# amoretti86/PSVO

Hardware: AMD Instinct MI355X
Metric: particle-steps/sec (higher is better)
Workload: dtype f32

## Files before the change

### psvo_amd/csrc/bsim_bwd2_impl.h

```cpp
#pragma once
#define PSVO_BSIM_BWD_V2_UNIT 1
#include "bsim_bwd_impl.h"

namespace psvo {
PSVO_TIMERS_DEFINE(bsim_bwd2)

__device__ __forceinline__ float ldf(const float* base, unsigned off) {
    return *reinterpret_cast<const float*>(reinterpret_cast<const char*>(base) + off);
}
__device__ __forceinline__ int ldi(const int32_t* base, unsigned off) {
    return *reinterpret_cast<const int32_t*>(reinterpret_cast<const char*>(base) + off);
}
__device__ __forceinline__ void stf(float* base, unsigned off, float v) {
    *reinterpret_cast<float*>(reinterpret_cast<char*>(base) + off) = v;
}

__device__ __forceinline__ float swap_add32(float lo, float hi) {
    asm volatile("s_nop 1\n\tv_permlane32_swap_b32 %0, %1" : "+v"(lo), "+v"(hi));
    return lo + hi;
}
__device__ __forceinline__ float swap_add16(float lo, float hi) {
    asm volatile("s_nop 1\n\tv_permlane16_swap_b32 %0, %1" : "+v"(lo), "+v"(hi));
    return lo + hi;
}
// ... 4 lines not shown
    v += dpp_mov<0x121, 0xF, 0xF, true>(v, v);
    return v;
}

__device__ __forceinline__ float rs_bit3(float lo, float hi) {
    float r;
    asm volatile("s_nop 1\n\t"
                 "v_add_f32_dpp %0, %1, %1 row_ror:8 row_mask:0xf bank_mask:0x3\n\t"
                 "v_add_f32_dpp %0, %2, %2 row_ror:8 row_mask:0xf bank_mask:0xc"
                 : "=&v"(r) : "v"(lo), "v"(hi));
    return r;
}
__device__ __forceinline__ float rs_bit2(float lo, float hi) {
    float r;
    asm volatile("s_nop 1\n\t"
                 "v_add_f32_dpp %0, %1, %1 row_shl:4 row_mask:0xf bank_mask:0x5\n\t"
                 "v_add_f32_dpp %0, %2, %2 row_shr:4 row_mask:0xf bank_mask:0xa"
                 : "=&v"(r) : "v"(lo), "v"(hi));
    return r;
}
template <int K>
__device__ __forceinline__ void row_reduce_scatter(const float (&v)[4 * K], float (&out)[K]) {
    float h[2 * K];
#pragma unroll
    for (int i = 0; i < 2 * K; ++i) h[i] = rs_bit3(v[i], v[2 * K + i]);
#pragma unroll
    for (int i = 0; i < K; ++i) out[i] = group_sum<4>(rs_bit2(h[i], h[K + i]));
}

typedef float f4v __attribute__((ext_vector_type(4)));
typedef __bf16 bf8v __attribute__((ext_vector_type(8)));

__device__ __forceinline__ void bf16_split3(float v, unsigned& h, unsigned& m, unsigned& l) {
    const unsigned hb = __float_as_uint(v) & 0xffff0000u;
    const float r = v - __uint_as_float(hb);
    const unsigned mb = __float_as_uint(r) & 0xffff0000u;
    const float r2 = r - __uint_as_float(mb);
    h = hb >> 16;
    m = mb >> 16;
    l = __float_as_uint(r2) >> 16;
}
__device__ __forceinline__ uint4 bf16x3_a(float v) {
    unsigned h, m, l;
    bf16_split3(v, h, m, l);
    return make_uint4(h | (h << 16), m | (h << 16), l | (m << 16), m | (l << 16));
}
__device__ __forceinline__ uint4 bf16x3_b(float v) {
    unsigned h, m, l;
    bf16_split3(v, h, m, l);
    return make_uint4(h | (m << 16), h | (l << 16), h | (m << 16), l | (m << 16));
}

template <int DX, int DY, int H, int M, int JM>
__global__ void __launch_bounds__(256, 2) bsim_bwd2_kernel(const BsimBwdArgs a) {
    using MQ = MlpLds<DX, H, DX, 1>;
    using MG = MlpLds<DX, H, DY, 1>;
    using AC = BAcc<DX, DY>;
    constexpr int PS = (JM == 3) ? 20 : (DX == 4 && JM == 0) ? 5 : BTileSlot<DX>::kFloats;
    constexpr int FO = (JM == 3) ? 16 : 0;
    constexpr int NA = DX + 1;
    constexpr int PART = 2;
    constexpr int G = M * PART;
    constexpr int CPW = 64 / G;
    constexpr int CM = CPW * M;
    constexpr int NF = DX + 2;
    constexpr int UVS = (2 * DX + 3) & ~3;
    constexpr int JC = (JM == 0 && DX == 4) ? 2 : (JM || DX >= 3) ? 4 : 8;
    constexpr bool RO = (DX == 4) && (JM == 0);
    constexpr bool kSplitTile = (DX == 4) && (JM == 0);
    static_assert(CM == 32 && (M % 4) == 0, "two lanes per (chain, m): M in {4, 8, 16, 32}");
    extern __shared__ __attribute__((aligned(16))) float smem[];

    const int tid = threadIdx.x, lane = tid & 63, wave = tid >> 6;
    constexpr int NTB = 256, nwv = 4;
    const int B = a.B, T = a.T, N = a.N;
    const int NP = ((N + 127) / 128) * 128;
    const int nch = NP / (16 * JC);
    const int b = blockIdx.y, blk = blockIdx.x, nblk = gridDim.x;
    constexpr int cpb = nwv * CPW;
    const int cl = lane / G, part = (lane / M) & 1, m = lane % M;
    const bool h0 = (part == 0);
    const int n_raw = blk * cpb + wave * CPW + cl;
    const bool valid = n_raw < N;
    const int n = valid ? n_raw : N - 1;
    const bool srow = valid && h0;
    const bool lead = srow && (m == 0);
    const int j16 = lane & 15, g = lane >> 4;

    float* wf = smem;
    float* wg = wf + MQ::kSize;
    float* wqi = wg + MG::kSize;
    float* tile = wqi + MQ::kSize;
    float* jacc = tile + 2 * NP * PS;
    float* xch = jacc + nwv * NA * NP;
    float* uvx = xch + nwv * NF * CM;
    float* red = uvx + nwv * CM * UVS;
    float* const xw = xch + wave * NF * CM;
    float* const uw = uvx + wave * CM * UVS;
    float* const ja = jacc + wave * NA * NP;

    MQ::load(wf, a.f, tid, NTB);
    MG::load(wg, a.g, tid, NTB);
    MQ::load(wqi, a.q1inv, tid, NTB);

    const float kappa = sqrtf(0.5f * kLog2e);
    float isf[DX], rp[DX], isfk[DX], isg[DY];
#pragma unroll
    for (int d = 0; d < DX; ++d) {
        isf[d] = 1.f / a.sig_f[d];
        rp[d] = isf[d] * kappa;
        isfk[d] = isf[d] / kappa;
    }
    float ikap2 = 1.f / (kappa * kappa);
#pragma unroll
    for (int e = 0; e < DY; ++e) isg[e] = 1.f / a.sig_g[e];
    float pc[DX], pic[DX], pi1[DX], pi2[DX];
#pragma unroll
    for (int d = 0; d < DX; ++d) {
        pi1[d] = 1.f / a.sig_q1inv[d];
        pi2[d] = 1.f / a.sig_bq2[d];
        pic[d] = pi1[d] + pi2[d];
        pc[d] = 1.f / pic[d];
    }
    float s_init[DX], is_init[DX], i_isig[DX], im[DX], mi[DX];
#pragma unroll
    for (int d = 0; d < DX; ++d) {
        s_init[d] = a.sig_init[d];
        is_init[d] = 1.f / s_init[d];
        i_isig[d] = 1.f / a.isig[d];
        im[d] = a.imean[b * DX + d];
        mi[d] = a.minit[b * DX + d];
    }
    if constexpr (DX <= 2) {
        keep_in_vgpr(isf); keep_in_vgpr(rp); keep_in_vgpr(isfk); keep_in_vgpr(isg); keep_in_vgpr(ikap2);
        keep_in_vgpr(pc); keep_in_vgpr(pic); keep_in_vgpr(pi1); keep_in_vgpr(pi2);
    }
    const float ninf = -__builtin_huge_valf();
    const float aw = valid ? a.dscore[(size_t)b * N + n] : 0.f;

    const unsigned NM = (unsigned)N * M;
    unsigned o_nm = 4u * ((unsigned)b * NM + n * M + m);
    unsigned o_dnm[DX], o_knm[DY], o_dn[DX];
#pragma unroll
    for (int d = 0; d < DX; ++d) {
        o_dnm[d] = 4u * (((unsigned)b * DX + d) * NM + n * M + m);
        o_dn[d] = 4u * (((unsigned)b * DX + d) * N + n);
    }
#pragma unroll
    for (int k = 0; k < DY; ++k) o_knm[k] = 4u * (((unsigned)b * DY + k) * NM + n * M + m);
    unsigned o_n = 4u * ((unsigned)b * N + n);
    unsigned o_d = 4u * ((unsigned)b * DX), o_k = 4u * ((unsigned)b * DY);
    const unsigned s_nm = 4u * B * NM, s_dnm = s_nm * DX, s_knm = s_nm * DY, s_dn = 4u * B * DX * N, s_n = 4u * B * N,
                   s_d = 4u * B * DX, s_k = 4u * B * DY;

    float st[DX + 1], st_l = 0.f;
    int st_t = 0;
    auto put_slot = [&](float* buf, int j, const float (&raw)[DX + 1], float l) {
        float F[DX];
#pragma unroll
        for (int d = 0; d < DX; ++d) F[d] = raw[d] * rp[d];
        const float W = j < N ? (raw[DX] - l) * kLog2e : ninf;
        if constexpr (JM == 3) {
            const float Wf = fmaxf(W, -1e30f);
            uint4* q = reinterpret_cast<uint4*>(buf + j * PS);
            q[0] = bf16x3_b(F[0]);
            q[1] = bf16x3_b(F[DX > 1 ? 1 : 0]);
            q[2] = bf16x3_b(Wf - (F[0] * F[0] + F[DX > 1 ? 1 : 0] * F[DX > 1 ? 1 : 0]));
            q[3] = bf16x3_b(1.f);
            *reinterpret_cast<float4*>(buf + j * PS + 16) = make_float4(F[0], F[DX > 1 ? 1 : 0], 0.f, 0.f);
        } else if constexpr (JM == 2) {
            *reinterpret_cast<float4*>(buf + j * PS) = make_float4(F[0], F[1], W - (F[0] * F[0] + F[DX > 1 ? 1 : 0] * F[DX > 1 ? 1 : 0]), 1.f);
        } else if constexpr (DX <= 3) {
            float4 v;
            v.x = F[0];
            v.y = DX > 1 ? F[DX > 1 ? 1 : 0] : 0.f;
            v.z = DX > 2 ? F[DX > 2 ? 2 : 0] : 0.f;
            v.w = W;
            *reinterpret_cast<float4*>(buf + j * PS) = v;
        } else if constexpr (kSplitTile) {
            *reinterpret_cast<float4*>(buf + 4 * j) = make_float4(F[0], F[1], F[2], F[3]);
            buf[4 * NP + j] = W;
        } else {
            *reinterpret_cast<float4*>(buf + j * PS) = make_float4(F[0], F[1], F[2], F[3]);
            *reinterpret_cast<float4*>(buf + j * PS + 4) = make_float4(W, 0.f, 0.f, 0.f);
        }
    };
    auto tile_entry = [&](const float* buf, int j, float (&F)[DX], float& W) {
        if constexpr (kSplitTile) {
            const float4 e = *reinterpret_cast<const float4*>(buf + 4 * j);
            F[0] = e.x; F[DX > 1 ? 1 : 0] = e.y; F[DX > 2 ? 2 : 0] = e.z; F[DX > 3 ? 3 : 0] = e.w;
            W = buf[4 * NP + j];
        } else {
            read_slot<DX>(buf + j * PS, F, W);
        }
    };
    static_assert(offsetof(BsimBwdArgs, logW) - offsetof(BsimBwdArgs, Fm) == 8 &&
                  offsetof(BsimBwdArgs, lse) - offsetof(BsimBwdArgs, Fm) == 16 && offsetof(BsimBwdArgs, Fm) % 32 == 0,
                  "BsimBwdArgs: forward-tile pointer block");
    auto get_slot = [&](int tt, int j, float (&raw)[DX + 1], const float* Fm, const float* logW) {
        const unsigned tb = (unsigned)tt * B + b;
        const unsigned jc = j < N ? j : N - 1;
#pragma unroll
        for (int d = 0; d < DX; ++d) raw[d] = ldf(Fm, 4u * ((tb * DX + d) * N + jc));
        raw[DX] = ldf(logW, 4u * (tb * N + jc));
    };
    float st2[DX + 1];
    const bool two_slots = (DX >= 3) && NP > NTB;
    auto stage_load = [&](int tt) {
        unsigned long long pt[4];
        arg_block<4>((unsigned)offsetof(BsimBwdArgs, Fm), pt);
        st_t = tt;
        st_l = ldf(reinterpret_cast<const float*>(pt[2]), 4u * ((unsigned)tt * B + b));
        if (tid < NP) get_slot(tt, tid, st, reinterpret_cast<const float*>(pt[0]), reinterpret_cast<const float*>(pt[1]));
        if (two_slots && tid + NTB < NP)
            get_slot(tt, tid + NTB, st2, reinterpret_cast<const float*>(pt[0]), reinterpret_cast<const float*>(pt[1]));
    };
    auto stage_store = [&](float* buf) {
        if (tid < NP) put_slot(buf, tid, st, st_l);
        if (two_slots && tid + NTB < NP) put_slot(buf, tid + NTB, st2, st_l);
        for (int j = tid + (two_slots ? 2 : 1) * NTB; j < NP; j += NTB) {
            float raw[DX + 1];
            get_slot(st_t, j, raw, PSVO_ARG(BsimBwdArgs, Fm), PSVO_ARG(BsimBwdArgs, logW));
            put_slot(buf, j, raw, st_l);
        }
    };
    if (T >= 2) {
        stage_load(0);
        stage_store(tile);
    }
    __syncthreads();

    constexpr bool kAccLds = (DX >= 3);
    constexpr int kRowsA = 2 * DX + DY, kRowsB = 5 * DX, kSlotsB = 8;
    float acc[kAccLds ? 1 : AC::kN];
    float* const accA = red + 16 + wave * (kRowsA * 32 + kRowsB * kSlotsB);
    float* const accB = accA + kRowsA * 32;
    auto acc_is_lead = [](int k) { return k < 4 * DX || (k >= 5 * DX && k < 6 * DX); };
    auto acc_row = [](int k) {
        return k < 4 * DX ? k : k < 5 * DX ? k - 4 * DX : k < 6 * DX ? 4 * DX + (k - 5 * DX)
               : k < 7 * DX ? DX + (k - 6 * DX) : 2 * DX + (k - 7 * DX);
    };
    const int s32 = cl * M + m;
    if constexpr (kAccLds) {
        for (int i = lane; i < kRowsA * 32 + kRowsB * kSlotsB; i += 64) accA[i] = 0.f;
    } else {
#pragma unroll
        for (int i = 0; i < AC::kN; ++i) acc[i] = 0.f;
    }
    auto acc_add = [&](int k, float v) {
        if constexpr (kAccLds) {
            if (acc_is_lead(k)) atomicAdd(&accB[acc_row(k) * kSlotsB + cl], v);
            else atomicAdd(&accA[acc_row(k) * 32 + s32], v);
        } else {
            acc[k] += v;
        }
    };
    float dX[DX];
#pragma unroll
    for (int d = 0; d < DX; ++d) dX[d] = 0.f;

    struct StepIn {
        float eps[DX], bm[DX], xp[DX], mu1[DX], y[DY], om, lam2;
        int sel;
    };
    static_assert(offsetof(BsimBwdArgs, dscore) - offsetof(BsimBwdArgs, obs) == 56 && offsetof(BsimBwdArgs, obs) % 64 == 0 &&
                  offsetof(BsimBwdArgs, eps_b) - offsetof(BsimBwdArgs, obs) == 8 &&
                  offsetof(BsimBwdArgs, bwX) - offsetof(BsimBwdArgs, obs) == 16 &&
                  offsetof(BsimBwdArgs, sel) - offsetof(BsimBwdArgs, obs) == 24 &&
                  offsetof(BsimBwdArgs, lam2_all) - offsetof(BsimBwdArgs, obs) == 32 &&
                  offsetof(BsimBwdArgs, om_all) - offsetof(BsimBwdArgs, obs) == 40 &&
                  offsetof(BsimBwdArgs, mu1_all) - offsetof(BsimBwdArgs, obs) == 48, "BsimBwdArgs: input pointer block");
    auto load_step = [&](bool lst, bool fst, StepIn& s) {
        unsigned long long pb[8];
        arg_block<8>((unsigned)offsetof(BsimBwdArgs, obs), pb);
        const float* const p_obs = reinterpret_cast<const float*>(pb[0]);
        const float* const p_eps = reinterpret_cast<const float*>(pb[1]);
        const float* const p_bwX = reinterpret_cast<const float*>(pb[2]);
        const int32_t* const p_sel = reinterpret_cast<const int32_t*>(pb[3]);
        const float* const p_lam2 = reinterpret_cast<const float*>(pb[4]);
        const float* const p_om = reinterpret_cast<const float*>(pb[5]);
        const float* const p_mu1 = reinterpret_cast<const float*>(pb[6]);
        const float* const p_bm = PSVO_ARG(BsimBwdArgs, bmu2);
        s.sel = ldi(p_sel, o_n);
#pragma unroll
        for (int d = 0; d < DX; ++d) {
            s.eps[d] = ldf(p_eps, o_dnm[d]);
            s.bm[d] = ldf(p_bm, o_d + 4u * d);
            s.xp[d] = lst ? 0.f : ldf(p_bwX, o_dn[d] + s_dn);
            s.mu1[d] = lst ? 0.f : ldf(p_mu1, o_dn[d]);
        }
#pragma unroll
        for (int k = 0; k < DY; ++k) s.y[k] = ldf(p_obs, o_k + 4u * k);
        s.om = ldf(p_om, o_nm);
        s.lam2 = fst ? 0.f : ldf(p_lam2, o_nm);
    };
    auto advance = [&]() {
        o_nm += s_nm; o_n += s_n; o_d += s_d; o_k += s_k;
#pragma unroll
        for (int d = 0; d < DX; ++d) { o_dnm[d] += s_dnm; o_dn[d] += s_dn; }
#pragma unroll
        for (int k = 0; k < DY; ++k) o_knm[k] += s_knm;
    };
    StepIn cur_in, nxt_in;
    load_step(T == 1, true, cur_in);

    phase_skew(a.skew);
    SEC_INIT(bsim_bwd2)
    for (int t = 0; t < T; ++t) {
        SEC(0);
        const bool first = (t == 0), last = (t == T - 1);
        const float* cur = tile + ((t + 1) & 1) * NP * PS;
        float* nxt = tile + (t & 1) * NP * PS;
        constexpr bool kLateTile = (DX == 4);
        if (!kLateTile && t + 1 < T && t >= 1) stage_load(t);
        advance();
        constexpr bool kLatePrefetch = (DX >= 3);
        if (!kLatePrefetch && t + 1 < T) load_step(t + 2 == T, false, nxt_in);
        SEC(1);

        float xp[DX], eps[DX], bm[DX], mu1[DX], mu[DX], x[DX], y[DY];
        const int sel = cur_in.sel;
#pragma unroll
        for (int d = 0; d < DX; ++d) {
            eps[d] = cur_in.eps[d];
            bm[d] = cur_in.bm[d];
            xp[d] = cur_in.xp[d];
            mu1[d] = cur_in.mu1[d];
            if (!last) {
                mu[d] = pc[d] * fmaf(pi1[d], mu1[d], pi2[d] * bm[d]);
                x[d] = fmaf(pc[d], eps[d], mu[d]);
            } else {
                mu[d] = mi[d];
                x[d] = fmaf(s_init[d], eps[d], mu[d]);
            }
        }
#pragma unroll
        for (int k = 0; k < DY; ++k) y[k] = cur_in.y[k];
        const float pi_m = valid ? exp2_fast(cur_in.om * kLog2e) : 0.f;
        const float issel = (m == sel) ? 1.f : 0.f;
        const float dphi = aw * pi_m;
        const float dlam = -aw * (issel - pi_m);

        float dxt[DX];
#pragma unroll
        for (int d = 0; d < DX; ++d) dxt[d] = h0 ? issel * dX[d] : 0.f;

        SEC(2);
        if (!first) {
            if (h0) {
#pragma unroll
                for (int d = 0; d < DX; ++d) xw[d * CM + cl * M + m] = x[d] * rp[d];
                xw[DX * CM + cl * M + m] = cur_in.lam2;
                xw[(DX + 1) * CM + cl * M + m] = dlam;
            }
            __builtin_amdgcn_fence(__ATOMIC_RELEASE, "wavefront");
            __builtin_amdgcn_wave_barrier();
            __builtin_amdgcn_fence(__ATOMIC_ACQUIRE, "wavefront");

            if constexpr (RO) {
#pragma unroll 1
                for (int r = 0; r < 2; ++r) {
                    const int it4 = 4 * (4 * r + g);
                    f2 xa[DX], xb[DX], Ua[DX], Ub[DX], Va[DX], Vb[DX];
#pragma unroll
                    for (int d = 0; d < DX; ++d) {
                        const float4 v = *reinterpret_cast<const float4*>(xw + d * CM + it4);
                        xa[d] = f2{v.x, v.y};
                        xb[d] = f2{v.z, v.w};
                        Ua[d] = Ub[d] = Va[d] = Vb[d] = f2{0.f, 0.f};
                    }
                    const float4 lq = *reinterpret_cast<const float4*>(xw + DX * CM + it4);
                    const float4 dl = *reinterpret_cast<const float4*>(xw + (DX + 1) * CM + it4);
                    const f2 lqa = f2{lq.x, lq.y}, lqb = f2{lq.z, lq.w};
                    const f2 dla = f2{dl.x, dl.y}, dlb = f2{dl.z, dl.w};
#pragma unroll 1
                    for (int c = 0; c < nch; ++c) {
                        float A2[JC][NA];
#pragma unroll
                        for (int jt = 0; jt < JC; ++jt) {
                            float F[DX], W;
                            tile_entry(cur, (c * JC + jt) * 16 + j16, F, W);
                            f2 ua[DX], ub[DX], la = f2{W, W}, lb = la;
#pragma unroll
                            for (int d = 0; d < DX; ++d) {
                                const f2 Fd = f2{F[d], F[d]};
                                ua[d] = xa[d] - Fd;
                                ub[d] = xb[d] - Fd;
                                la = pk_fma(-ua[d], ua[d], la);
                                lb = pk_fma(-ub[d], ub[d], lb);
                            }
                            la -= lqa;
                            lb -= lqb;
                            const f2 pa = f2{exp2_fast(la.x), exp2_fast(la.y)}, pb = f2{exp2_fast(lb.x), exp2_fast(lb.y)};
                            const f2 ca = dla * pa, cb = dlb * pb;
#pragma unroll
                            for (int d = 0; d < DX; ++d) {
                                const f2 pua = pa * ua[d], pub = pb * ub[d];
                                Ua[d] += pua;
                                Ub[d] += pub;
                                Va[d] = pk_fma(pua, ua[d], Va[d]);
                                Vb[d] = pk_fma(pub, ub[d], Vb[d]);
                            }
                            const f2 cs = ca + cb;
                            A2[jt][DX] = cs.x + cs.y;
#pragma unroll
                            for (int d = 0; d < DX; ++d) {
                                const f2 ad = pk_fma(cb, ub[d], ca * ua[d]);
                                A2[jt][d] = ad.x + ad.y;
                            }
                        }
                        static_assert(JC == 2, "rounds-outer flush: two tiles per chunk");
#pragma unroll
                        for (int e = 0; e < NA; ++e) {
                            float v = swap_add32(A2[0][e], A2[1][e]);
                            v += xor_lane<16>(v);
                            if ((g & 1) == 0) {
                                float* dst = ja + e * NP + (c * JC + (g >> 1)) * 16 + j16;
                                *dst = (r == 0) ? v : *dst + v;
                            }
                        }
                    }
                    float vv[4 * 2 * DX], o[UVS];
#pragma unroll
                    for (int d = 0; d < DX; ++d) {
                        vv[0 * 2 * DX + d] = Ua[d].x; vv[1 * 2 * DX + d] = Ua[d].y;
                        vv[2 * 2 * DX + d] = Ub[d].x; vv[3 * 2 * DX + d] = Ub[d].y;
                        vv[0 * 2 * DX + DX + d] = Va[d].x; vv[1 * 2 * DX + DX + d] = Va[d].y;
                        vv[2 * 2 * DX + DX + d] = Vb[d].x; vv[3 * 2 * DX + DX + d] = Vb[d].y;
                    }
                    float red2[2 * DX];
                    row_reduce_scatter<2 * DX>(vv, red2);
#pragma unroll
                    for (int e = 0; e < UVS; ++e) o[e] = e < 2 * DX ? red2[e < 2 * DX ? e : 0] : 0.f;
                    if ((j16 & 3) == 0) {
                        float* dst = uw + (4 * (4 * r + g) + (j16 >> 2)) * UVS;
#pragma unroll
                        for (int e = 0; e < UVS; e += 4)
                            *reinterpret_cast<float4*>(dst + e) = make_float4(o[e], o[e + 1], o[e + 2], o[e + 3]);
                    }
                }
            } else {
            f2 Ua[2][DX], Ub[2][DX], Va[2][DX], Vb[2][DX];
#pragma unroll
            for (int r = 0; r < 2; ++r)
#pragma unroll
                for (int d = 0; d < DX; ++d) Ua[r][d] = Ub[r][d] = Va[r][d] = Vb[r][d] = f2{0.f, 0.f};

            for (int c = 0; c < nch; ++c) {
                float A2[JC][NA];
                f4v D4[JC];
#pragma unroll
                for (int jt = 0; jt < JC; ++jt) {
#pragma unroll
                    for (int e = 0; e < NA; ++e) A2[jt][e] = 0.f;
                    D4[jt] = f4v{0.f, 0.f, 0.f, 0.f};
                }
                const float* cbase = cur + (c * 16 * JC + j16) * PS;
#pragma unroll
                for (int r = 0; r < 2; ++r) {
                    const int it4 = 4 * (4 * r + g);
                    f2 xa[DX], xb[DX];
#pragma unroll
                    for (int d = 0; d < DX; ++d) {
                        const float4 v = *reinterpret_cast<const float4*>(xw + d * CM + it4);
                        xa[d] = f2{v.x, v.y};
                        xb[d] = f2{v.z, v.w};
                    }
                    const float4 lq = *reinterpret_cast<const float4*>(xw + DX * CM + it4);
                    const float4 dl = *reinterpret_cast<const float4*>(xw + (DX + 1) * CM + it4);
                    const f2 lqa = f2{lq.x, lq.y}, lqb = f2{lq.z, lq.w};
                    const f2 dla = f2{dl.x, dl.y}, dlb = f2{dl.z, dl.w};
// ... 57 lines not shown
                        }
                    } else
#pragma unroll
                    for (int jt = 0; jt < JC; ++jt) {
                        float F[DX], W;
                        if constexpr (kSplitTile) tile_entry(cur, (c * JC + jt) * 16 + j16, F, W);
                        else read_slot<DX>(cbase + jt * 16 * PS, F, W);
                        f2 ua[DX], ub[DX], la = f2{W, W}, lb = la;
#pragma unroll
                        for (int d = 0; d < DX; ++d) {
                            const f2 Fd = f2{F[d], F[d]};
                            ua[d] = xa[d] - Fd;
                            ub[d] = xb[d] - Fd;
                            la = pk_fma(-ua[d], ua[d], la);
                            lb = pk_fma(-ub[d], ub[d], lb);
                        }
                        la -= lqa;
                        lb -= lqb;
                        const f2 pa = f2{exp2_fast(la.x), exp2_fast(la.y)}, pb = f2{exp2_fast(lb.x), exp2_fast(lb.y)};
                        const f2 ca = dla * pa, cb = dlb * pb;
#pragma unroll
                        for (int d = 0; d < DX; ++d) {
                            const f2 pua = pa * ua[d], pub = pb * ub[d];
                            Ua[r][d] += pua;
                            Ub[r][d] += pub;
                            Va[r][d] = pk_fma(pua, ua[d], Va[r][d]);
                            Vb[r][d] = pk_fma(pub, ub[d], Vb[r][d]);
                        }
                        if constexpr (JM != 1) {
                            const f2 cs = ca + cb;
                            A2[jt][DX] += cs.x + cs.y;
#pragma unroll
                            for (int d = 0; d < DX; ++d) {
                                const f2 ad = pk_fma(cb, ub[d], ca * ua[d]);
                                A2[jt][d] += ad.x + ad.y;
                            }
                        } else {
                            D4[jt] = __builtin_amdgcn_mfma_f32_16x16x4f32(xop[0], ca.x, D4[jt], 0, 0, 0);
                            D4[jt] = __builtin_amdgcn_mfma_f32_16x16x4f32(xop[1], ca.y, D4[jt], 0, 0, 0);
                            D4[jt] = __builtin_amdgcn_mfma_f32_16x16x4f32(xop[2], cb.x, D4[jt], 0, 0, 0);
                            D4[jt] = __builtin_amdgcn_mfma_f32_16x16x4f32(xop[3], cb.y, D4[jt], 0, 0, 0);
                        }
                    }
                }
                if constexpr (JM != 1) {
                    float v[JC][NA];
#pragma unroll
                    for (int jt = 0; jt < JC; ++jt)
#pragma unroll
                        for (int e = 0; e < NA; ++e) v[jt][e] = A2[jt][e];
#pragma unroll
                    for (int jt = 0; jt < JC / 2; ++jt)
#pragma unroll
                        for (int e = 0; e < NA; ++e) v[jt][e] = swap_add32(v[jt][e], v[jt + JC / 2][e]);
#pragma unroll
                    for (int jt = 0; jt < JC / 4; ++jt)
#pragma unroll
                        for (int e = 0; e < NA; ++e) v[jt][e] = swap_add16(v[jt][e], v[jt + JC / 4][e]);
                    const int jt0 = (JC / 2) * (g >> 1) + (JC / 4) * (g & 1);
#pragma unroll
                    for (int jt = 0; jt < JC / 4; ++jt) {
                        if constexpr (JM >= 2) {
                            const float2 F2 = *reinterpret_cast<const float2*>(cbase + (jt0 + jt) * 16 * PS + FO);
                            v[jt][0] = fmaf(-F2.x, v[jt][DX], v[jt][0]);
                            v[jt][DX > 1 ? 1 : 0] = fmaf(-F2.y, v[jt][DX], v[jt][DX > 1 ? 1 : 0]);
                        }
#pragma unroll
                        for (int e = 0; e < NA; ++e) ja[e * NP + (c * JC + jt0 + jt) * 16 + j16] = v[jt][e];
                    }
                } else {
                    if (g == 0 || DX > 3) {
#pragma unroll
                        for (int jt = 0; jt < JC; ++jt) {
                            float F[DX], W;
                            read_slot<DX>(cbase + jt * 16 * PS, F, W);
                            (void)W;
                            const int j = (c * JC + jt) * 16 + j16;
                            if constexpr (DX <= 3) {
                                const float sc = D4[jt][DX];
#pragma unroll
                                for (int d = 0; d < DX; ++d) ja[d * NP + j] = D4[jt][d] - F[d] * sc;
                                ja[DX * NP + j] = sc;
                            } else {
                                const float sc = __shfl(D4[jt][0], 16 + j16);
                                if (g == 0) {
#pragma unroll
                                    for (int d = 0; d < DX; ++d) ja[d * NP + j] = D4[jt][d] - F[d] * sc;
                                    ja[DX * NP + j] = sc;
                                }
                            }
                        }
                    }
                }
            }
#pragma unroll
            for (int r = 0; r < 2; ++r) {
                float vv[4 * 2 * DX], o[UVS];
#pragma unroll
                for (int d = 0; d < DX; ++d) {
                    vv[0 * 2 * DX + d] = Ua[r][d].x; vv[1 * 2 * DX + d] = Ua[r][d].y;
                    vv[2 * 2 * DX + d] = Ub[r][d].x; vv[3 * 2 * DX + d] = Ub[r][d].y;
                    vv[0 * 2 * DX + DX + d] = Va[r][d].x; vv[1 * 2 * DX + DX + d] = Va[r][d].y;
                    vv[2 * 2 * DX + DX + d] = Vb[r][d].x; vv[3 * 2 * DX + DX + d] = Vb[r][d].y;
                }
                float red2[2 * DX];
                row_reduce_scatter<2 * DX>(vv, red2);
#pragma unroll
                for (int e = 0; e < UVS; ++e) o[e] = e < 2 * DX ? red2[e < 2 * DX ? e : 0] : 0.f;
                if ((j16 & 3) == 0) {
                    float* dst = uw + (4 * (4 * r + g) + (j16 >> 2)) * UVS;
#pragma unroll
                    for (int e = 0; e < UVS; e += 4)
                        *reinterpret_cast<float4*>(dst + e) = make_float4(o[e], o[e + 1], o[e + 2], o[e + 3]);
                }
            }
            }
            __builtin_amdgcn_fence(__ATOMIC_RELEASE, "wavefront");
            __builtin_amdgcn_wave_barrier();
            __builtin_amdgcn_fence(__ATOMIC_ACQUIRE, "wavefront");
            SEC(3);
            if (h0) {
                float uv[UVS];
#pragma unroll
                for (int e = 0; e < UVS; e += 4) {
                    const float4 q4 = *reinterpret_cast<const float4*>(uw + (cl * M + m) * UVS + e);
                    uv[e] = q4.x; uv[e + 1] = q4.y; uv[e + 2] = q4.z; uv[e + 3] = q4.w;
                }
                if constexpr (JM >= 2) {
#pragma unroll
                    for (int d = 0; d < DX; ++d) {
                        const float xs = x[d] * rp[d], r1 = uv[d], r2 = uv[DX + d];
                        uv[d] = xs - r1;
                        uv[DX + d] = fmaf(xs, xs - 2.f * r1, r2);
                    }
                }
#pragma unroll
                for (int d = 0; d < DX; ++d) {
                    dxt[d] -= dlam * uv[d] * isfk[d];
                    acc_add(AC::kSf + d, dlam * (uv[DX + d] * ikap2 - 1.f) * isf[d]);
                }
            }
        } else {
#pragma unroll
            for (int d = 0; d < DX; ++d) {
                const float z = (x[d] - im[d]) * i_isig[d];
                const float tz = dphi * z * i_isig[d];
                if (h0) {
                    dxt[d] -= tz;
                    acc_add(AC::kSiota + d, dphi * (z * z - 1.f) * i_isig[d]);
                }
            }
        }

        if (kLatePrefetch && t + 1 < T) load_step(t + 2 == T, false, nxt_in);
        if (kLateTile && t + 1 < T && t >= 1) stage_load(t);
        SEC(4);
        float dxp_part[DX];
#pragma unroll
        for (int d = 0; d < DX; ++d) dxp_part[d] = 0.f;
        {
            float dFo[DX];
#pragma unroll
            for (int d = 0; d < DX; ++d) dFo[d] = 0.f;
            if (!last) {
                float fmx[DX];
                MQ::template eval_part<PART>(wf, part, x, fmx);
#pragma unroll
                for (int d = 0; d < DX; ++d) fmx[d] += xor_lane<M>(fmx[d]);
#pragma unroll
                for (int d = 0; d < DX; ++d) {
                    const float z = (xp[d] - fmx[d]) * isf[d];
                    dFo[d] = dphi * z * isf[d];
                    if (h0) {
                        dxp_part[d] = -dFo[d];
                        acc_add(AC::kSf + d, dphi * (z * z - 1.f) * isf[d]);
                    }
                }
                MQ::template bwd_input_part<PART>(wf, part, x, dFo, dxt);
            }
            static_assert(offsetof(BsimBwdArgs, dFt) - offsetof(BsimBwdArgs, xt) == 8 &&
                          offsetof(BsimBwdArgs, dGt) - offsetof(BsimBwdArgs, xt) == 16 &&
                          offsetof(BsimBwdArgs, dmu1) - offsetof(BsimBwdArgs, xt) == 24 && offsetof(BsimBwdArgs, xt) % 32 == 0,
                          "BsimBwdArgs: row pointer block");
            unsigned long long pr[4];
            arg_block<4>((unsigned)offsetof(BsimBwdArgs, xt), pr);
            if (srow) {
#pragma unroll
                for (int d = 0; d < DX; ++d) {
                    stf(reinterpret_cast<float*>(pr[1]), o_dnm[d] - s_dnm, dFo[d]);
                    stf(reinterpret_cast<float*>(pr[0]), o_dnm[d] - s_dnm, x[d]);
                }
            }
            float gm[DY], dGo[DY];
            MG::template eval_part<PART>(wg, part, x, gm);
#pragma unroll
            for (int k = 0; k < DY; ++k) gm[k] += xor_lane<M>(gm[k]);
#pragma unroll
            for (int k = 0; k < DY; ++k) {
                float dmean = 1.f;
                if (a.emission) { dmean = emis_dmean(gm[k]); gm[k] = emis_mean(gm[k]); }
                const float z = (y[k] - gm[k]) * isg[k];
                dGo[k] = dphi * z * isg[k] * dmean;
                if (h0) acc_add(AC::kSg + k, dphi * (z * z - 1.f) * isg[k]);
                if (srow) stf(reinterpret_cast<float*>(pr[2]), o_knm[k] - s_knm, dGo[k]);
            }
            MG::template bwd_input_part<PART>(wg, part, x, dGo, dxt);
        }

        SEC(5);
        float dmu[DX], sce[DX], dxp[DX], dim[DX];
#pragma unroll
        for (int d = 0; d < DX; ++d) {
            const float v3 = (first && h0) ? dphi * (x[d] - im[d]) * i_isig[d] * i_isig[d] : 0.f;
            dmu[d] = group_sum<G>(dxt[d]);
            sce[d] = group_sum<G>(dxt[d] * eps[d]);
            dxp[d] = group_sum<G>(dxp_part[d]);
            dim[d] = first ? group_sum<G>(v3) : 0.f;
        }
        float outv[DX];
        if (!last) {
            float dmu1[DX];
#pragma unroll
            for (int d = 0; d < DX; ++d) {
                dmu1[d] = dmu[d] * pc[d] * pi1[d];
                outv[d] = dmu[d] * pc[d] * pi2[d];
                if (lead) {
                    stf(PSVO_ARG(BsimBwdArgs, dmu1), o_dn[d] - s_dn, dmu1[d]);
                    acc_add(AC::kSc + d, sce[d] + aw * pic[d]);
                    acc_add(AC::kSmm1 + d, dmu[d] * mu1[d]);
                    acc_add(AC::kSmb + d, dmu[d] * bm[d]);
                    acc_add(AC::kSmm + d, dmu[d] * mu[d]);
                }
            }
            {
                constexpr int kQS = (H / 4 < G) ? H / 4 : G;
                float dq[DX];
#pragma unroll
                for (int d = 0; d < DX; ++d) dq[d] = 0.f;
                MQ::template bwd_input_part<kQS>(wqi, (lane % G) & (kQS - 1), xp, dmu1, dq);
#pragma unroll
                for (int d = 0; d < DX; ++d) dxp[d] += group_sum<kQS>(dq[d]);
            }
        } else {
#pragma unroll
            for (int d = 0; d < DX; ++d) {
                outv[d] = dmu[d];
                if (lead) {
                    stf(PSVO_ARG(BsimBwdArgs, dmu1), o_dn[d] - s_dn, 0.f);
                    acc_add(AC::kSinit + d, sce[d] + aw * is_init[d]);
                }
            }
        }
#pragma unroll
        for (int d = 0; d < DX; ++d) dX[d] = dxp[d];
        if (lead) {
#pragma unroll
            for (int d = 0; d < DX; ++d) {
                stf(PSVO_ARG(BsimBwdArgs, dbmu2_rows), o_dn[d] - s_dn, last ? 0.f : outv[d]);
                if (last) PSVO_ARG(BsimBwdArgs, dminit_rows)[((size_t)b * DX + d) * N + n] = outv[d];
                if (first) PSVO_ARG(BsimBwdArgs, dimean_rows)[((size_t)b * DX + d) * N + n] = dim[d];
            }
        }
        SEC(6);
        __syncthreads();
        const size_t tb = (size_t)t * B + b;
        if (!first) {
            const size_t tbm = tb - B;
            float* const pF = PSVO_ARG(BsimBwdArgs, dFm_part) + (tbm * nblk + blk) * DX * N;
            float* const pW = PSVO_ARG(BsimBwdArgs, dlogW_part) + (tbm * nblk + blk) * N;
            for (int j = tid; j < N; j += NTB) {
#pragma unroll
                for (int d = 0; d < NA; ++d) {
                    const float* col = jacc + d * NP + j;
                    const float a0 = col[0], a1 = col[NA * NP], a2 = col[2 * NA * NP], a3 = col[3 * NA * NP];
                    const float s = (a0 + a1) + (a2 + a3);
                    if (d < DX) pF[d * N + j] = s * isfk[d < DX ? d : 0];
                    else pW[j] = s;
                }
            }
        }
        if (last) {
            float* const pF = PSVO_ARG(BsimBwdArgs, dFm_part) + (tb * nblk + blk) * DX * N;
            float* const pW = PSVO_ARG(BsimBwdArgs, dlogW_part) + (tb * nblk + blk) * N;
            for (int j = tid; j < N; j += NTB) {
#pragma unroll
                for (int d = 0; d < DX; ++d) pF[d * N + j] = 0.f;
                pW[j] = 0.f;
            }
        }
        SEC(7);
        if (t + 1 < T && t >= 1) stage_store(nxt);
        cur_in = nxt_in;
        __syncthreads();
        SEC(8);
    }

    for (int i = 0; i < AC::kN; ++i) {
        float v = 0.f;
        if constexpr (kAccLds) {
            if (acc_is_lead(i)) v = lane < kSlotsB ? accB[acc_row(i) * kSlotsB + lane] : 0.f;
            else v = lane < 32 ? accA[acc_row(i) * 32 + lane] : 0.f;
        } else {
#pragma unroll
            for (int k = 0; k < AC::kN; ++k) v = (k == i) ? acc[k] : v;
        }
        v = wave_sum(v);
        if (lane == 0) red[wave] = v;
        __syncthreads();
        if (tid == 0) {
            float s = 0.f;
            for (int w = 0; w < nwv; ++w) s += red[w];
            a.sacc_part[((size_t)b * nblk + blk) * AC::kN + i] = s;
        }
        __syncthreads();
    }
}

static inline void bsim2_geometry(int N, int M, int& cpb, int& nblk) {
    cpb = 4 * (64 / (2 * M));
    nblk = (N + cpb - 1) / cpb;
}

static inline bool bsim2_supported(int B, int T, int N, int M, int Dx, int Dy) {
    if (pick_m(M, [](auto) { return PSVO_OK; }) != PSVO_OK) return false;
    const long long big = (long long)T * B * (Dx > Dy ? Dx : Dy) * N * M * 4;
    return big < (1ll << 32);
}

template <int DX, int DY, int H, int M>
static int launch_bsim_bwd2(const BsimBwdArgs& a, const BsimBwdOut& o, int jm, hipStream_t stream) {
    using MQ = MlpLds<DX, H, DX, 1>;
    using MG = MlpLds<DX, H, DY, 1>;
    const int PS = (jm == 3 && DX == 2) ? 20 : (DX == 4) ? 5 : BTileSlot<DX>::kFloats;
    constexpr int UVS = (2 * DX + 3) & ~3;
    int cpb, nblk;
    bsim2_geometry(a.N, M, cpb, nblk);
    const int NP = ((a.N + 127) / 128) * 128;
    const size_t lds = sizeof(float) * (2 * MQ::kSize + MG::kSize + 2 * (size_t)NP * PS + 4 * (size_t)(DX + 1) * NP +
                                        4 * (DX + 2) * 32 + 4 * 32 * UVS + 16 +
                                        (DX >= 3 ? 4 * ((2 * DX + DY) * 32 + 5 * DX * 8) : 0));
    if (lds > 160 * 1024) return PSVO_ERR_UNSUPPORTED;
    BsimBwdArgs as = a;
    as.skew = (int)(2560.0 * NP / 128.0 * (3 * DX + 4) / 10.0 * g_tune_skew_pct / 100.0);
    clear_hip_error();
    if (jm == 3 && DX == 2) {
        if constexpr (DX == 2)
            hipLaunchKernelGGL((bsim_bwd2_kernel<DX, DY, H, M, 3>), dim3(nblk, a.B), dim3(256), lds, stream, as);
    } else if (jm == 2 && DX == 2) {
        if constexpr (DX == 2)
            hipLaunchKernelGGL((bsim_bwd2_kernel<DX, DY, H, M, 2>), dim3(nblk, a.B), dim3(256), lds, stream, as);
    } else if (jm == 1 && DX == 2) {
        if constexpr (DX == 2)
            hipLaunchKernelGGL((bsim_bwd2_kernel<DX, DY, H, M, 1>), dim3(nblk, a.B), dim3(256), lds, stream, as);
    } else {
        hipLaunchKernelGGL((bsim_bwd2_kernel<DX, DY, H, M, 0>), dim3(nblk, a.B), dim3(256), lds, stream, as);
    }
    (void)o;
    return launch_status();
}

template <int DX>
int bb2_dispatch_dy(const BsimBwdArgs& a, const BsimBwdOut& o, int Dy, int H, int M, int jm, hipStream_t s) {
    return dispatch_dy_h_m(Dy, H, M, [&](auto dy, auto h, auto m) __attribute__((visibility("hidden"))) {
        return launch_bsim_bwd2<DX, dy(), h(), m()>(a, o, jm, s); });
}

}
```

### psvo_amd/csrc/common.h

```cpp
#pragma once
#include <cstddef>
#include <type_traits>
#include <hip/hip_runtime.h>
#include <stdint.h>

#include "../../include/psvo_hip.h"

#ifndef PSVO_L
#define PSVO_L 1
#endif
#if PSVO_L == 1
#define PSVO_LNS l1
#define PSVO_ENTRY(name) extern "C" int name
#define PSVO_L2_DECL(name) extern "C" __attribute__((visibility("hidden"))) decltype(name) name##_l2;
#elif PSVO_L == 2
#define PSVO_LNS l2
#define PSVO_ENTRY(name) extern "C" __attribute__((visibility("hidden"))) int name##_l2
#define PSVO_L2_DECL(name)
#else
#error "PSVO_L must be 1 or 2"
#endif

namespace psvo {

constexpr float kLog2e = 1.4426950408889634f;
constexpr float kLn2 = 0.6931471805599453f;
constexpr float kHalfLog2Pi = 0.9189385332046727f;
constexpr int kWave = 64;

extern thread_local hipError_t g_last_hip_error;
inline void clear_hip_error() { (void)hipGetLastError(); }
inline int launch_status() {
    const hipError_t e = hipGetLastError();
    if (e != hipSuccess) g_last_hip_error = e;
    return e == hipSuccess ? PSVO_OK : PSVO_ERR_HIP;
}

inline bool desc_layers_ok(const psvo_desc* d) { return !d || (d->layers >= 0 && d->layers <= 2); }

extern int g_tune_l2_split;
extern int g_tune_filter_bwd_scan;

extern int g_tune_skew_pct;

__device__ __forceinline__ void phase_skew(int cycles) {
    unsigned hw;
    asm volatile("s_getreg_b32 %0, hwreg(HW_REG_HW_ID)" : "=s"(hw));
    if (cycles > 0 && ((hw >> 16) & 1u)) {
        for (int i = 0; i < cycles; i += 64 * 32) __builtin_amdgcn_s_sleep(32);
    }
}

inline bool mlp_layers_ok(const psvo_mlp* m) { return PSVO_L == 1 || !m || (m->Wh && m->bh); }

template <int V, int... Vs, class F>
static inline int pick(int v, F&& f) {
    if (v == V) return f(std::integral_constant<int, V>{});
    if constexpr (sizeof...(Vs) > 0) return pick<Vs...>(v, f);
    else return PSVO_ERR_UNSUPPORTED;
}
template <class F> static inline int pick_dx(int Dx, F&& f) { return pick<2, 3, 4>(Dx, f); }
template <class F> static inline int pick_dy(int Dy, F&& f) { return pick<1, 2>(Dy, f); }
template <class F> static inline int pick_m(int M, F&& f) { return pick<4, 8, 16, 32>(M, f); }
inline namespace PSVO_LNS {
template <class F> static inline int pick_h(int H, F&& f) {
#if PSVO_L == 1
    return pick<16, 32, 64>(H, f);
#else
    return pick<32, 64>(H, f);
#endif
}

template <class F> static inline int dispatch_dy_h(int Dy, int H, F&& f) {
    return pick_dy(Dy, [&](auto dy) { return pick_h(H, [&](auto h) { return f(dy, h); }); });
}
template <class F> static inline int dispatch_dy_h_m(int Dy, int H, int M, F&& f) {
    return dispatch_dy_h(Dy, H, [&](auto dy, auto h) { return pick_m(M, [&](auto m) { return f(dy, h, m); }); });
}
template <class F> static inline int dispatch_shape(int Dx, int Dy, int H, F&& f) {
    return pick_dx(Dx, [&](auto dx) { return dispatch_dy_h(Dy, H, [&](auto dy, auto h) { return f(dx, dy, h); }); });
}
template <class F> static inline int dispatch_shape_m(int Dx, int Dy, int H, int M, F&& f) {
    return pick_dx(Dx, [&](auto dx) { return dispatch_dy_h_m(Dy, H, M, [&](auto dy, auto h, auto m) { return f(dx, dy, h, m); }); });
}
}

static inline int wr_cluster(int B, int N, int M) {
    int K = 8;
    while (K > 1 && ((long long)B * K > 256 || N < 4 * K || (N + K - 1) / K * (K - 1) >= N)) K >>= 1;
    (void)M;
    return K;
}

#ifdef PSVO_SECTION_TIMERS
#define PSVO_TIMERS_DEFINE(name)                                                                        \
    __device__ unsigned long long g_sec_##name[32];                                                       \
    extern "C" int psvo_debug_timers_##name(unsigned long long* out, int reset) {                         \
        if (hipMemcpyFromSymbol(out, HIP_SYMBOL(g_sec_##name), 32 * sizeof(unsigned long long)) != hipSuccess) \
            return -1;                                                                                    \
        if (reset) {                                                                                      \
            unsigned long long z[32] = {0};                                                               \
            if (hipMemcpyToSymbol(HIP_SYMBOL(g_sec_##name), z, sizeof(z)) != hipSuccess) return -1;       \
        }                                                                                                 \
        return 0;                                                                                         \
    }
#define SEC_INIT(name)                                                                          \
    unsigned long long* const _sec = g_sec_##name;                                              \
    const bool _rec = (blockIdx.x == 0 && blockIdx.y == 0 && threadIdx.x == 0);                 \
    unsigned long long _tp = clock64();
#define SEC(i)                                   \
    do {                                         \
        const unsigned long long _tn = clock64(); \
        if (_rec) _sec[i] += _tn - _tp;          \
        _tp = _tn;                               \
    } while (0)
#else
#define PSVO_TIMERS_DEFINE(name)
#define SEC_INIT(name)
#define SEC(i)
#endif

__device__ __forceinline__ float exp2_fast(float x) { return __builtin_amdgcn_exp2f(x); }
__device__ __forceinline__ float log2_fast(float x) { return __builtin_amdgcn_logf(x); }

typedef float f2 __attribute__((ext_vector_type(2)));
__device__ __forceinline__ f2 pk_fma(f2 a, f2 b, f2 c) { return __builtin_elementwise_fma(a, b, c); }
__device__ __forceinline__ f2 pk_max(f2 a, f2 b) { return __builtin_elementwise_max(a, b); }
template <int HALF>
__device__ __forceinline__ f2 pk_fma_bcast(f2 a, f2 b, f2 c) {
    f2 d;
    if constexpr (HALF == 0)
        asm("v_pk_fma_f32 %0, %1, %2, %3 op_sel_hi:[0,1,1]" : "=v"(d) : "v"(a), "v"(b), "v"(c));
    else
        asm("v_pk_fma_f32 %0, %1, %2, %3 op_sel:[1,0,0] op_sel_hi:[1,1,1]" : "=v"(d) : "v"(a), "v"(b), "v"(c));
    return d;
}

__device__ __forceinline__ void keep_in_vgpr(float& x) { asm volatile("" : "+v"(x)); }
template <int K>
__device__ __forceinline__ void keep_in_vgpr(float (&x)[K]) {
#pragma unroll
    for (int i = 0; i < K; ++i) asm volatile("" : "+v"(x[i]));
}

template <class T>
__device__ __forceinline__ T* arg_ptr(unsigned byte_off) {
    asm volatile("" : "+s"(byte_off));
    typedef const char __attribute__((address_space(4))) * kptr;
    const kptr kp = (kptr)__builtin_amdgcn_kernarg_segment_ptr();
    typedef T* const __attribute__((address_space(4))) * pptr;
    return *(pptr)(kp + byte_off);
}
template <int NPTR>
__device__ __forceinline__ void arg_block(unsigned byte_off, unsigned long long (&out)[NPTR]) {
    static_assert(NPTR == 2 || NPTR == 4 || NPTR == 8, "pointer block of 2, 4 or 8");
    asm volatile("" : "+s"(byte_off));
    typedef const char __attribute__((address_space(4))) * kptr;
    const kptr kp = (kptr)__builtin_amdgcn_kernarg_segment_ptr();
    typedef unsigned long long vec_t __attribute__((ext_vector_type(NPTR)));
    typedef const vec_t __attribute__((address_space(4))) * vptr;
    const vec_t v = *(vptr)(kp + byte_off);
#pragma unroll
    for (int i = 0; i < NPTR; ++i) out[i] = v[i];
}
#define PSVO_ARG(args_type, field) \
    ::psvo::arg_ptr<std::remove_pointer_t<decltype(args_type::field)>>((unsigned)offsetof(args_type, field))

__device__ __forceinline__ float emis_mean(float r) { return (r > 20.f ? r : log1pf(expf(r))) + 1e-6f; }
__device__ __forceinline__ float emis_dmean(float r) { return 1.f / (1.f + expf(-r)); }

template <int DIN, int H, int DOUT, int L = 1>
struct MlpLds;

template <int DIN, int H, int DOUT>
struct MlpLds<DIN, H, DOUT, 1> {
    static constexpr int kW1 = 0;
    static constexpr int kB1 = DIN * H;
    static constexpr int kW2 = kB1 + H;
    static constexpr int kB2 = kW2 + DOUT * H;
    static constexpr int kSize = kB2 + ((DOUT + 3) & ~3);

    __device__ static void load(float* __restrict__ w, const psvo_mlp& p, int tid, int nthreads) {
        for (int i = tid; i < DIN * H; i += nthreads) w[kW1 + i] = p.W1[i];
        for (int i = tid; i < H; i += nthreads) w[kB1 + i] = p.b1[i];
        for (int i = tid; i < DOUT * H; i += nthreads) {
            const int o = i / H, k = i - o * H;
            w[kW2 + i] = p.W2[k * DOUT + o];
        }
        for (int i = tid; i < ((DOUT + 3) & ~3); i += nthreads) w[kB2 + i] = i < DOUT ? p.b2[i] : 0.f;
    }

    __device__ __forceinline__ static void group4(const float* __restrict__ w, int k, const float (&x)[DIN],
                                                  f2 (&acc)[DOUT]) {
        const float4 b = *reinterpret_cast<const float4*>(w + kB1 + k);
        f2 ha = f2{b.x, b.y}, hb = f2{b.z, b.w};
#pragma unroll
        for (int i = 0; i < DIN; ++i) {
            const float4 wi = *reinterpret_cast<const float4*>(w + kW1 + i * H + k);
            const f2 xi = f2{x[i], x[i]};
            ha = pk_fma(xi, f2{wi.x, wi.y}, ha);
            hb = pk_fma(xi, f2{wi.z, wi.w}, hb);
        }
        const f2 zero = f2{0.f, 0.f};
        ha = pk_max(ha, zero);
        hb = pk_max(hb, zero);
#pragma unroll
        for (int o = 0; o < DOUT; ++o) {
            const float4 wo = *reinterpret_cast<const float4*>(w + kW2 + o * H + k);
            acc[o] = pk_fma(ha, f2{wo.x, wo.y}, acc[o]);
            acc[o] = pk_fma(hb, f2{wo.z, wo.w}, acc[o]);
        }
    }

    template <bool ROLLED = false>
    __device__ __forceinline__ static void eval(const float* __restrict__ w, const float (&x)[DIN],
                                                float (&out)[DOUT]) {
        f2 acc[DOUT];
#pragma unroll
        for (int o = 0; o < DOUT; ++o) acc[o] = f2{w[kB2 + o], 0.f};
        if constexpr (ROLLED && (H % 8 == 0) && (H > 8)) {
#pragma unroll 1
            for (int k = 0; k < H; k += 8) {
                group4(w, k, x, acc);
                group4(w, k + 4, x, acc);
            }
        } else {
#pragma unroll
            for (int k = 0; k < H; k += 4) group4(w, k, x, acc);
        }
#pragma unroll
        for (int o = 0; o < DOUT; ++o) out[o] = acc[o].x + acc[o].y;
    }

    template <int S, int PB = 0>
    __device__ __forceinline__ static void eval_part(const float* __restrict__ w, int part, const float (&x)[DIN],
                                                     float (&out)[DOUT]) {
        constexpr int HP = H / S;
        static_assert(HP % 4 == 0, "hidden slice must be a multiple of 4");
        const float* wp = w + part * HP;
        f2 acc[DOUT];
#pragma unroll
        for (int o = 0; o < DOUT; ++o) acc[o] = f2{part == 0 ? w[kB2 + o] : 0.f, 0.f};
#pragma unroll
        for (int k = 0; k < HP; k += 4) group4(wp, k, x, acc);
#pragma unroll
        for (int o = 0; o < DOUT; ++o) out[o] = acc[o].x + acc[o].y;
    }

    __device__ __forceinline__ static void bwd_group4(const float* __restrict__ w, int k, const float (&x)[DIN],
                                                      const float (&dout)[DOUT], f2 (&dxa)[DIN]) {
        const float4 b = *reinterpret_cast<const float4*>(w + kB1 + k);
        f2 pa = f2{b.x, b.y}, pb = f2{b.z, b.w};
        f2 wa[DIN], wb[DIN];
#pragma unroll
        for (int i = 0; i < DIN; ++i) {
            const float4 wi = *reinterpret_cast<const float4*>(w + kW1 + i * H + k);
            wa[i] = f2{wi.x, wi.y};
            wb[i] = f2{wi.z, wi.w};
            const f2 xi = f2{x[i], x[i]};
            pa = pk_fma(xi, wa[i], pa);
            pb = pk_fma(xi, wb[i], pb);
        }
        f2 da = f2{0.f, 0.f}, db = da;
#pragma unroll
        for (int o = 0; o < DOUT; ++o) {
            const float4 wo = *reinterpret_cast<const float4*>(w + kW2 + o * H + k);
            const f2 go = f2{dout[o], dout[o]};
            da = pk_fma(go, f2{wo.x, wo.y}, da);
            db = pk_fma(go, f2{wo.z, wo.w}, db);
        }
        da = f2{pa.x > 0.f ? da.x : 0.f, pa.y > 0.f ? da.y : 0.f};
        db = f2{pb.x > 0.f ? db.x : 0.f, pb.y > 0.f ? db.y : 0.f};
#pragma unroll
        for (int i = 0; i < DIN; ++i) {
            dxa[i] = pk_fma(da, wa[i], dxa[i]);
            dxa[i] = pk_fma(db, wb[i], dxa[i]);
        }
    }

    template <int S, int PB = 0>
    __device__ __forceinline__ static void bwd_input_part(const float* __restrict__ w, int part, const float (&x)[DIN],
                                                          const float (&dout)[DOUT], float (&dx)[DIN]) {
        constexpr int HP = H / S;
        const float* wp = w + part * HP;
        f2 dxa[DIN];
#pragma unroll
        for (int i = 0; i < DIN; ++i) dxa[i] = f2{dx[i], 0.f};
#pragma unroll
// ... 371 lines not shown
```

Measured before the change: 240.9 million.

## Stage per-step inputs through a cooperative LDS slab instead of per-lane global loads

```diff
diff --git a/psvo_amd/csrc/bsim_bwd2_impl.h b/psvo_amd/csrc/bsim_bwd2_impl.h
--- a/psvo_amd/csrc/bsim_bwd2_impl.h
+++ b/psvo_amd/csrc/bsim_bwd2_impl.h
@@ -180,6 +180,62 @@
     unsigned o_d = 4u * ((unsigned)b * DX), o_k = 4u * ((unsigned)b * DY);
     const unsigned s_nm = 4u * B * NM, s_dnm = s_nm * DX, s_knm = s_nm * DY, s_dn = 4u * B * DX * N, s_n = 4u * B * N,
                    s_d = 4u * B * DX, s_k = 4u * B * DY;
+
+    constexpr bool kSlab = (DX <= 3);
+    constexpr int kBig = (DX + 2) * 128;
+    constexpr int kSm = 2 * DX * cpb + cpb + DX + DY;
+    static_assert(cpb * M == 128 && (!kSlab || kSm <= NTB), "step record: one dword per thread covers the small values");
+    float* const slab = red + 16 + (DX >= 3 ? nwv * ((2 * DX + DY) * 32 + 5 * DX * 8) : 0);
+    size_t lp4 = 0, lp1 = 0;
+    unsigned ls4 = 0, ls1 = 0;
+    bool big = false, big_lam2 = false, sml = false, sml_next = false;
+    if constexpr (kSlab) {
+        unsigned long long pb[8];
+        arg_block<8>((unsigned)offsetof(BsimBwdArgs, obs), pb);
+        const int n0 = blk * cpb;
+        {
+            const int r = tid >> 5, e = 4 * (tid & 31);
+            const int nc = min(n0 + e / M, N - 1);
+            const unsigned in_row = 4u * ((unsigned)nc * M + e % M);
+            big = r < DX + 2;
+            big_lam2 = (r == DX + 1);
+            const unsigned long long base = r < DX ? pb[1] : r == DX ? pb[5] : pb[4];
+            const unsigned row = r < DX ? ((unsigned)b * DX + r) * NM : (unsigned)b * NM;
+            lp4 = base + (4u * row + in_row);
+            ls4 = r < DX ? s_dnm : s_nm;
+        }
+        {
+            const int s = NTB - 1 - tid;
+            constexpr int kX = DX * cpb, kMu = 2 * DX * cpb, kSel = kMu + cpb, kBm = kSel + DX;
+            sml = s < kSm;
+            sml_next = s < kX;
+            const int q = s < kX ? s : s < kMu ? s - kX : 0;
+            const int c = s < kMu ? q % cpb : s < kSel ? s - kMu : 0;
+            const int nc = min(n0 + c, N - 1);
+            const unsigned o_xm = 4u * (((unsigned)b * DX + q / cpb) * N + nc);
+            const unsigned long long bm_base = reinterpret_cast<unsigned long long>(PSVO_ARG(BsimBwdArgs, bmu2));
+            const int dbm = min(max(s - kSel, 0), DX - 1), ky = min(max(s - kBm, 0), DY - 1);
+            const unsigned long long base = s < kX ? pb[2] : s < kMu ? pb[6] : s < kSel ? pb[3] : s < kBm ? bm_base : pb[0];
+            const unsigned off = s < kX ? o_xm + s_dn : s < kMu ? o_xm : s < kSel ? 4u * ((unsigned)b * N + nc)
+                                 : s < kBm ? 4u * ((unsigned)b * DX + dbm) : 4u * ((unsigned)b * DY + ky);
+            lp1 = base + off;
+            ls1 = s < kMu ? s_dn : s < kSel ? s_n : s < kBm ? s_d : s_k;
+        }
+    }
+    f4 sg4 = f4{0.f, 0.f, 0.f, 0.f};
+    unsigned sg1 = 0u;
+    auto slab_load = [&](bool lst) {
+        if (big) sg4 = ldg_f4(lp4);
+        if (sml) sg1 = ldg_u32((lst && sml_next) ? lp1 - ls1 : lp1);
+    };
+    auto slab_store = [&](bool lst, bool fst) {
+        if (big) *reinterpret_cast<f4*>(slab + 4 * tid) = (fst && big_lam2) ? f4{0.f, 0.f, 0.f, 0.f} : sg4;
+        if (sml) reinterpret_cast<unsigned*>(slab)[kBig + (NTB - 1 - tid)] = (lst && sml_next) ? 0u : sg1;
+    };
+    if constexpr (kSlab) {
+        slab_load(T == 1);
+        slab_store(T == 1, true);
+    }
 
     float st[DX + 1], st_l = 0.f;
     int st_t = 0;
@@ -328,9 +384,26 @@
         for (int d = 0; d < DX; ++d) { o_dnm[d] += s_dnm; o_dn[d] += s_dn; }
 #pragma unroll
         for (int k = 0; k < DY; ++k) o_knm[k] += s_knm;
+        if constexpr (kSlab) { lp4 += ls4; lp1 += ls1; }
     };
     StepIn cur_in, nxt_in;
-    load_step(T == 1, true, cur_in);
+    if constexpr (!kSlab) load_step(T == 1, true, cur_in);
+    auto slab_read = [&](StepIn& s) {
+        const int cw = wave * CPW + cl, ce = cw * M + m;
+        const float* const sm = slab + kBig;
+#pragma unroll
+        for (int d = 0; d < DX; ++d) {
+            s.eps[d] = slab[d * 128 + ce];
+            s.xp[d] = sm[d * cpb + cw];
+            s.mu1[d] = sm[(DX + d) * cpb + cw];
+            s.bm[d] = sm[(2 * DX + 1) * cpb + d];
+        }
+#pragma unroll
+        for (int k = 0; k < DY; ++k) s.y[k] = sm[(2 * DX + 1) * cpb + DX + k];
+        s.om = slab[DX * 128 + ce];
+        s.lam2 = slab[(DX + 1) * 128 + ce];
+        s.sel = __float_as_int(sm[2 * DX * cpb + cw]);
+    };
 
     phase_skew(a.skew);
     SEC_INIT(bsim_bwd2)
@@ -343,8 +416,13 @@
         if (!kLateTile && t + 1 < T && t >= 1) stage_load(t);
         advance();
         constexpr bool kLatePrefetch = (DX >= 3);
-        if (!kLatePrefetch && t + 1 < T) load_step(t + 2 == T, false, nxt_in);
+        auto prefetch = [&]() {
+            if constexpr (kSlab) slab_load(t + 2 == T);
+            else load_step(t + 2 == T, false, nxt_in);
+        };
+        if (!kLatePrefetch && t + 1 < T) prefetch();
         SEC(1);
+        if constexpr (kSlab) slab_read(cur_in);
 
         float xp[DX], eps[DX], bm[DX], mu1[DX], mu[DX], x[DX], y[DY];
         const int sel = cur_in.sel;
@@ -708,7 +786,7 @@
             }
         }
 
-        if (kLatePrefetch && t + 1 < T) load_step(t + 2 == T, false, nxt_in);
+        if (kLatePrefetch && t + 1 < T) prefetch();
         if (kLateTile && t + 1 < T && t >= 1) stage_load(t);
         SEC(4);
         float dxp_part[DX];
@@ -846,7 +924,11 @@
         }
         SEC(7);
         if (t + 1 < T && t >= 1) stage_store(nxt);
-        cur_in = nxt_in;
+        if constexpr (kSlab) {
+            if (t + 1 < T) slab_store(t + 2 == T, false);
+        } else {
+            cur_in = nxt_in;
+        }
         __syncthreads();
         SEC(8);
     }
@@ -894,7 +976,8 @@
     const int NP = ((a.N + 127) / 128) * 128;
     const size_t lds = sizeof(float) * (2 * MQ::kSize + MG::kSize + 2 * (size_t)NP * PS + 4 * (size_t)(DX + 1) * NP +
                                         4 * (DX + 2) * 32 + 4 * 32 * UVS + 16 +
-                                        (DX >= 3 ? 4 * ((2 * DX + DY) * 32 + 5 * DX * 8) : 0));
+                                        (DX >= 3 ? 4 * ((2 * DX + DY) * 32 + 5 * DX * 8) : 0) +
+                                        (DX <= 3 ? (DX + 2) * 128 + (((2 * DX + 1) * (128 / M) + DX + DY + 3) & ~3) : 0));
     if (lds > 160 * 1024) return PSVO_ERR_UNSUPPORTED;
     BsimBwdArgs as = a;
     as.skew = (int)(2560.0 * NP / 128.0 * (3 * DX + 4) / 10.0 * g_tune_skew_pct / 100.0);
diff --git a/psvo_amd/csrc/common.h b/psvo_amd/csrc/common.h
--- a/psvo_amd/csrc/common.h
+++ b/psvo_amd/csrc/common.h
@@ -134,6 +134,15 @@
     else
         asm("v_pk_fma_f32 %0, %1, %2, %3 op_sel:[1,0,0] op_sel_hi:[1,1,1]" : "=v"(d) : "v"(a), "v"(b), "v"(c));
     return d;
+}
+
+typedef float f4 __attribute__((ext_vector_type(4)));
+typedef f4 __attribute__((aligned(4))) f4_a4;
+__device__ __forceinline__ f4 ldg_f4(size_t addr) {
+    return *reinterpret_cast<const f4_a4 __attribute__((address_space(1)))*>(addr);
+}
+__device__ __forceinline__ unsigned ldg_u32(size_t addr) {
+    return *reinterpret_cast<const unsigned __attribute__((address_space(1)))*>(addr);
 }
 
 __device__ __forceinline__ void keep_in_vgpr(float& x) { asm volatile("" : "+v"(x)); }
```

Result: no change. 243.2 million (median of 6 runs) (+1.0%).
